# callmeray/PointMVSNet

Hardware: AMD Instinct MI355X
Metric: depth-maps/sec (DTU 640x512, 3 src views, 2 flow iters) (higher is better)
Workload: dtype f32

## Files before the change

pointmvsnet_amd/csrc/conv3d.hip:

```cpp
#include <stdlib.h>

#include "pf_common.h"
#include "pf_bn_resolve.h"

namespace {

typedef float f32x4 __attribute__((ext_vector_type(4)));

struct ConvGeom {
  int Cin, Cout, Di, Hi, Wi, Do, Ho, Wo;
  int ID, IH, IW, IWP, plane;
  int tiles_d, tiles_h, tiles_w;
  int aff_mode, sps, aff_off;
  const float* in_scale;
  const float* in_shift;
  pf_bn_job in_bn;
};

template <int STRIDE, int TD>
struct Stage {
  static constexpr int ID = (TD - 1) * STRIDE + 3;
  static constexpr int IH = 3 * STRIDE + 3;
  static constexpr int IW = 15 * STRIDE + 3;
  static constexpr int IWP = IW + 1;
  static constexpr int RAW = ID * IH * IWP;
  static constexpr int WANT = STRIDE == 1 ? 16 : 17;
  static constexpr int PLANE = RAW + ((WANT - RAW % 32) + 32) % 32;
  static constexpr int ELEMS = ID * IH * IW;
  static constexpr int NXR = (ELEMS + 63) / 64;
};

template <int NT, int STRIDE, int TD, int MINW>
__global__ __launch_bounds__(256, MINW) void conv3d_k3_kernel(const float* __restrict__ x, const float* __restrict__ wp,
                                                        float* __restrict__ y, ConvGeom g,
                                                        double* __restrict__ partials) {
  using St = Stage<STRIDE, TD>;
  constexpr int ID = St::ID, IH = St::IH, IW = St::IW, IWP = St::IWP, PLANE = St::PLANE;
  constexpr int ELEMS = St::ELEMS, NXR = St::NXR;
  constexpr int NCP = NT * 16;
  constexpr int WSZ = 27 * 4 * NCP;
  constexpr int NWR = (WSZ + 255) / 256;
  constexpr int XS = 4 * PLANE;
  extern __shared__ __attribute__((aligned(16))) float lds[];
  float* xs0 = lds;
  float* ws0 = lds + 2 * XS;
  float* tile = lds;
  double* red = reinterpret_cast<double*>(tile + 4 * NCP * 17 + ((4 * NCP * 17) & 1));

  const int tid = threadIdx.x;
  const int wave = __builtin_amdgcn_readfirstlane(tid >> 6), lane = tid & 63;
  const int li = lane & 15, lk = lane >> 4;
  unsigned xb_, xn_;
  pf_xcd_xy<PF_XCD_CONV3D>(xb_, xn_);
  const int n = (int)xn_, bx = (int)xb_;
  const int plane_i = g.Hi * g.Wi, vol_i = plane_i * g.Di;
  const int64_t plane_o = (int64_t)g.Ho * g.Wo, vol_o = plane_o * g.Do;
  const float* xb = x + (int64_t)n * g.Cin * vol_i;
  float* yb = y + (int64_t)n * g.Cout * vol_o;
  const int cgroups = g.Cin >> 2;

  double ssum[NT], ssq[NT];
#pragma unroll
  for (int t = 0; t < NT; ++t) ssum[t] = ssq[t] = 0.0;

  float* aff = lds + g.aff_off;
  if (g.aff_mode == 1) {
    const int stat = n / g.sps;
    for (int e = tid; e < 2 * g.Cin; e += 256)
      aff[e] = e < g.Cin ? g.in_scale[(int64_t)stat * g.Cin + e] : g.in_shift[(int64_t)stat * g.Cin + e - g.Cin];
  } else if (g.aff_mode == 2) {
    pf_bn_resolve<256>(g.in_bn, n / g.sps, aff, aff + g.Cin, reinterpret_cast<double*>(lds));
  }

  const int total = g.tiles_d * g.tiles_h * g.tiles_w;
  for (int item = bx; item < total; item += gridDim.x) {
    const int tw = item % g.tiles_w;
    const int rest = item / g.tiles_w;
    const int th = rest % g.tiles_h;
    const int td = rest / g.tiles_h;
    const int od0 = td * TD, oh0 = th * 4, ow0 = tw * 16;
    const int id0 = od0 * STRIDE - 1, ih0 = oh0 * STRIDE - 1, iw0 = ow0 * STRIDE - 1;

    unsigned gofs[NXR];
    unsigned okmask = 0;
#pragma unroll
    for (int r = 0; r < NXR; ++r) {
      const int e = lane + 64 * r;
      const int row = e / IW, col = e - row * IW;
      const int dz = row / IH, hy = row - dz * IH;
      const int id = id0 + dz, ih = ih0 + hy, iw = iw0 + col;
      const bool ok = e < ELEMS && id >= 0 && id < g.Di && ih >= 0 && ih < g.Hi && iw >= 0 && iw < g.Wi;
      gofs[r] = ok ? (unsigned)(id * plane_i + ih * g.Wi + iw) : 0u;
      okmask |= (ok ? 1u : 0u) << r;
    }

    float rx[NXR], rw[NWR];
    auto load_group = [&](int cg) {
      const float* src = xb + (int64_t)(cg * 4 + wave) * vol_i;
#pragma unroll
      for (int r = 0; r < NXR; ++r) rx[r] = src[gofs[r]];
      const float* wsrc = wp + (int64_t)cg * WSZ;
#pragma unroll
      for (int r = 0; r < NWR; ++r) {
        const int e = tid + 256 * r;
        rw[r] = (256 * (r + 1) <= WSZ || e < WSZ) ? wsrc[e] : 0.0f;
      }
    };
    auto store_group = [&](int buf, int cg) {
      float* xs = xs0 + buf * XS + wave * PLANE;
      float* ws = ws0 + buf * WSZ;
      float sa = 1.0f, sb = 0.0f;
      if (g.aff_mode) {
        sa = aff[cg * 4 + wave];
        sb = aff[g.Cin + cg * 4 + wave];
      }
#pragma unroll
      for (int r = 0; r < NXR; ++r) {
        const int e = lane + 64 * r;
        float v = rx[r];
        if (g.aff_mode) v = fmaxf(fmaf(v, sa, sb), 0.0f);
        if (64 * (r + 1) <= ELEMS || e < ELEMS) xs[e + e / IW] = ((okmask >> r) & 1u) ? v : 0.0f;
      }
#pragma unroll
      for (int r = 0; r < NWR; ++r) {
        const int e = tid + 256 * r;
        if (256 * (r + 1) <= WSZ || e < WSZ) ws[e] = rw[r];
      }
    };

    f32x4 acc[TD][NT];
#pragma unroll
    for (int d = 0; d < TD; ++d)
#pragma unroll
      for (int t = 0; t < NT; ++t) acc[d][t] = (f32x4){0.0f, 0.0f, 0.0f, 0.0f};

    __syncthreads();
    load_group(0);
    store_group(0, 0);
    __syncthreads();
    for (int cg = 0; cg < cgroups; ++cg) {
      const int buf = cg & 1;
      if (cg + 1 < cgroups) load_group(cg + 1);
      const float* xs = xs0 + buf * XS + lk * PLANE + (wave * STRIDE) * IWP + li * STRIDE;
      const float* ws = ws0 + buf * WSZ + lk * NCP + li;
#pragma unroll
      for (int kd = 0; kd < 3; ++kd) {
#pragma unroll
        for (int kh = 0; kh < 3; ++kh) {
#pragma unroll
          for (int kw = 0; kw < 3; ++kw) {
            const int tap = (kd * 3 + kh) * 3 + kw;
            float b[NT];
#pragma unroll
            for (int t = 0; t < NT; ++t) b[t] = ws[tap * 4 * NCP + 16 * t];
#pragma unroll
            for (int d = 0; d < TD; ++d) {
              const float a = xs[((d * STRIDE + kd) * IH + kh) * IWP + kw];
#pragma unroll
              for (int t = 0; t < NT; ++t) acc[d][t] = __builtin_amdgcn_mfma_f32_16x16x4f32(a, b[t], acc[d][t], 0, 0, 0);
            }
          }
        }
      }
      if (cg + 1 < cgroups) store_group(buf ^ 1, cg + 1);
      __syncthreads();
    }

    const int oh = oh0 + wave;
    float* tl = tile + wave * NCP * 17;
#pragma unroll
    for (int d = 0; d < TD; ++d) {
      const int od = od0 + d;
      const bool row_ok = oh < g.Ho && od < g.Do;
#pragma unroll
      for (int t = 0; t < NT; ++t) {
        float s = 0.0f, q = 0.0f;
#pragma unroll
        for (int r = 0; r < 4; ++r) {
          const int pos = lk * 4 + r;
          const float v = acc[d][t][r];
          tl[(16 * t + li) * 17 + pos] = v;
          if (row_ok && ow0 + pos < g.Wo) {
            s += v;
            q += v * v;
          }
        }
        s += __shfl_xor(s, 16);
        q += __shfl_xor(q, 16);
        s += __shfl_xor(s, 32);
        q += __shfl_xor(q, 32);
        ssum[t] += (double)s;
        ssq[t] += (double)q;
      }
      __builtin_amdgcn_wave_barrier();
      if (row_ok) {
        for (int e = lane; e < NCP * 16; e += 64) {
          const int co = e >> 4, pos = e & 15;
          if (co < g.Cout && ow0 + pos < g.Wo)
            yb[(int64_t)co * vol_o + (int64_t)od * plane_o + (int64_t)oh * g.Wo + ow0 + pos] = tl[co * 17 + pos];
        }
      }
      __builtin_amdgcn_wave_barrier();
    }
  }

  if (partials != nullptr) {
#pragma unroll
    for (int t = 0; t < NT; ++t) {
      if (lane < 16) {
        red[((wave * NCP) + 16 * t + lane) * 2 + 0] = ssum[t];
        red[((wave * NCP) + 16 * t + lane) * 2 + 1] = ssq[t];
      }
    }
    __syncthreads();
    if (tid < g.Cout) {
      double s = 0.0, q = 0.0;
#pragma unroll
      for (int w = 0; w < 4; ++w) {
        s += red[((w * NCP) + tid) * 2 + 0];
        q += red[((w * NCP) + tid) * 2 + 1];
      }
      double* o = partials + (((int64_t)n * gridDim.x + bx) * g.Cout + tid) * 2;
      o[0] = s;
      o[1] = q;
    }
  }
}

template <int COUT>
__global__ __launch_bounds__(256) void conv3d_k3_few_kernel(const float* __restrict__ x, const float* __restrict__ w,
                                                            float* __restrict__ y, int Cin, int D, int H, int W) {
  extern __shared__ __attribute__((aligned(16))) float wl[];
  for (int e = threadIdx.x; e < COUT * Cin * 27; e += 256) wl[e] = w[e];
  __syncthreads();
  const int64_t plane = (int64_t)H * W, vol = plane * D;
  const int64_t i = (int64_t)blockIdx.x * 256 + threadIdx.x;
  const int n = blockIdx.y;
  if (i >= vol) return;
  const int od = (int)(i / plane);
  const int rem = (int)(i - (int64_t)od * plane);
  const int oh = rem / W, ow = rem - oh * W;
  float acc[COUT];
#pragma unroll
  for (int c = 0; c < COUT; ++c) acc[c] = 0.0f;
  const float* xb = x + (int64_t)n * Cin * vol;
  for (int ci = 0; ci < Cin; ++ci) {
    const float* xc = xb + (int64_t)ci * vol;
#pragma unroll
    for (int kd = 0; kd < 3; ++kd) {
      const int id = od + kd - 1;
      const bool dok = id >= 0 && id < D;
#pragma unroll
      for (int kh = 0; kh < 3; ++kh) {
        const int ih = oh + kh - 1;
        const bool hok = dok && ih >= 0 && ih < H;
        const float* row = xc + (int64_t)id * plane + (int64_t)ih * W;
#pragma unroll
        for (int kw = 0; kw < 3; ++kw) {
          const int iw = ow + kw - 1;
          const float v = (hok && iw >= 0 && iw < W) ? row[iw] : 0.0f;
#pragma unroll
          for (int c = 0; c < COUT; ++c) acc[c] = fmaf(v, wl[(c * Cin + ci) * 27 + (kd * 3 + kh) * 3 + kw], acc[c]);
        }
      }
    }
  }
#pragma unroll
  for (int c = 0; c < COUT; ++c) y[((int64_t)n * COUT + c) * vol + i] = acc[c];
}

ConvGeom make_geom(int64_t Cin, int64_t Cout, int64_t Di, int64_t Hi, int64_t Wi, int stride, int td) {
  ConvGeom g;
  g.Cin = (int)Cin;
  g.Cout = (int)Cout;
  g.Di = (int)Di;
  g.Hi = (int)Hi;
  g.Wi = (int)Wi;
  g.Do = (int)((Di - 1) / stride + 1);
  g.Ho = (int)((Hi - 1) / stride + 1);
  g.Wo = (int)((Wi - 1) / stride + 1);
  g.ID = (td - 1) * stride + 3;
  g.IH = 3 * stride + 3;
  g.IW = 15 * stride + 3;
  g.IWP = g.IW + 1;
  const int raw = g.ID * g.IH * g.IWP;
  const int want = stride == 1 ? 16 : 17;
  g.plane = raw + ((want - raw % 32) + 32) % 32;
  g.tiles_d = (g.Do + td - 1) / td;
  g.tiles_h = (g.Ho + 3) / 4;
  g.tiles_w = (g.Wo + 15) / 16;
  g.aff_mode = 0;
  g.sps = 1;
  g.aff_off = 0;
  g.in_scale = g.in_shift = nullptr;
  g.in_bn = pf_bn_job{};
  return g;
}

constexpr size_t kMaxLds = 80 * 1024;

size_t lds_work_bytes(const ConvGeom& g, int NT) {
  const int NCP = NT * 16;
  const size_t staging = sizeof(float) * (size_t)(2 * 4 * g.plane + 2 * 27 * 4 * NCP);
  const size_t epilogue = sizeof(float) * (size_t)(4 * NCP * 17 + 1) + sizeof(double) * (size_t)(4 * NCP * 2);
  const size_t m = staging > epilogue ? staging : epilogue;
  return (m + 15) / 16 * 16;
}
size_t lds_bytes_for(const ConvGeom& g, int NT) {
  return lds_work_bytes(g, NT) + sizeof(float) * 2 * (size_t)g.Cin;
}

int pick_td(int64_t Cin, int64_t Cout, int64_t Di, int64_t Hi, int64_t Wi, int stride) {
  const int NT = (int)((Cout + 15) / 16);
  int best = 0;
  for (int td = (stride == 1 && NT > 1) ? 4 : 2; td >= 1; td >>= 1) {
    const ConvGeom g = make_geom(Cin, Cout, Di, Hi, Wi, stride, td);
    if (lds_bytes_for(g, NT) > kMaxLds) continue;
    best = td;
    if ((int64_t)g.tiles_d * g.tiles_h * g.tiles_w >= 512) return td;
  }
  return best;
}

int blocks_for(const ConvGeom& g) {
  const int64_t total = (int64_t)g.tiles_d * g.tiles_h * g.tiles_w;
#ifndef PF_CONV3D_CAP
#define PF_CONV3D_CAP 2048
#endif
  if (total <= PF_CONV3D_CAP) return (int)total;
  const int64_t per = (total + PF_CONV3D_CAP - 1) / PF_CONV3D_CAP;
  return (int)((total + per - 1) / per);
}

template <int NT, int STRIDE, int TD, int MINW>
int launch(const float* x, const float* wp, float* y, const ConvGeom& g, int64_t N, double* partials,
           hipStream_t s) {
  const size_t lds_bytes = lds_bytes_for(g, NT);
  if (lds_bytes > kMaxLds) return PF_ERR_UNSUPPORTED;
  ConvGeom gk = g;
  gk.aff_off = (int)(lds_work_bytes(g, NT) / sizeof(float));
  if (lds_bytes > 64 * 1024) {
    static std::atomic<unsigned long long> done{0};
    const int rc = pf_allow_big_lds(reinterpret_cast<const void*>(&conv3d_k3_kernel<NT, STRIDE, TD, MINW>),
                                    (int)kMaxLds, done);
    if (rc != PF_OK) return rc;
  }
  dim3 grid((unsigned)blocks_for(g), (unsigned)N);
  hipLaunchKernelGGL((conv3d_k3_kernel<NT, STRIDE, TD, MINW>), grid, dim3(256), lds_bytes, s, x, wp, y, gk, partials);
  return pf_launch_status();
}

template <int NT, int STRIDE, int TD>
int launch_w(const float* x, const float* wp, float* y, const ConvGeom& g, int64_t N, double* partials,
             hipStream_t s) {
  constexpr int kDefault = (NT == 1 && STRIDE == 1 && TD == 2) ? 4 : 2;
  return launch<NT, STRIDE, TD, kDefault>(x, wp, y, g, N, partials, s);
}

template <int NT, int STRIDE>
int launch_td(int td, const float* x, const float* wp, float* y, const ConvGeom& g, int64_t N, double* partials,
              hipStream_t s) {
  if constexpr (STRIDE == 1) {
    if (td == 4) return launch_w<NT, STRIDE, 4>(x, wp, y, g, N, partials, s);
  }
  if (td == 2) return launch_w<NT, STRIDE, 2>(x, wp, y, g, N, partials, s);
  return launch_w<NT, STRIDE, 1>(x, wp, y, g, N, partials, s);
}

}

extern "C" {

int pf_conv3d_blocks(int64_t Cin, int64_t Cout, int64_t Di, int64_t Hi, int64_t Wi, int stride) {
  if (Cin <= 0 || Cout <= 0 || Di <= 0 || Hi <= 0 || Wi <= 0 || (stride != 1 && stride != 2)) return 0;
  const int td = pick_td(Cin, Cout, Di, Hi, Wi, stride);
  if (td == 0) return 0;
  return blocks_for(make_geom(Cin, Cout, Di, Hi, Wi, stride, td));
}

int pf_conv3d_k3_f32(const float* x, const float* wp, float* y, int64_t N, int64_t Cin, int64_t Cout, int64_t Di,
                     int64_t Hi, int64_t Wi, int stride, const float* in_scale, const float* in_shift,
                     const pf_bn_job* in_bn, int samples_per_stat, double* partials, void* stream) {
  PF_REQUIRE(N >= 0 && Cin >= 4 && Cout >= 1 && Di >= 1 && Hi >= 1 && Wi >= 1 && N <= 65535);
  PF_REQUIRE(stride == 1 || stride == 2);
  PF_REQUIRE(samples_per_stat >= 1 && (in_scale == nullptr) == (in_shift == nullptr));
  PF_REQUIRE(in_bn == nullptr || in_scale == nullptr);
  if (in_bn != nullptr && N > 0) {
    PF_REQUIRE(N % samples_per_stat == 0);
    const int rc = pf_bn_in_check(in_bn, (int)Cin, (int)(N / samples_per_stat));
    if (rc != PF_OK) return rc;
  }
  if ((Cin % 4) != 0 || Cout > 32) return PF_ERR_UNSUPPORTED;
  PF_REQUIRE(Cin * Di * Hi * Wi <= INT32_MAX);
  if (N == 0) return PF_OK;
  PF_REQUIRE(x && wp && y);
  const int td = pick_td(Cin, Cout, Di, Hi, Wi, stride);
  if (td == 0) return PF_ERR_UNSUPPORTED;
  ConvGeom g = make_geom(Cin, Cout, Di, Hi, Wi, stride, td);
  g.aff_mode = in_bn ? 2 : (in_scale ? 1 : 0);
  g.sps = samples_per_stat;
  g.in_scale = in_scale;
  g.in_shift = in_shift;
  if (in_bn) g.in_bn = *in_bn;
  hipStream_t s = (hipStream_t)stream;
  const int NT = (int)((Cout + 15) / 16);
  if (stride == 1)
    return NT == 1 ? launch_td<1, 1>(td, x, wp, y, g, N, partials, s) : launch_td<2, 1>(td, x, wp, y, g, N, partials, s);
  return NT == 1 ? launch_td<1, 2>(td, x, wp, y, g, N, partials, s) : launch_td<2, 2>(td, x, wp, y, g, N, partials, s);
}

int pf_conv3d_k3_few_f32(const float* x, const float* w, float* y, int64_t N, int64_t Cin, int64_t Cout, int64_t D,
                         int64_t H, int64_t W, void* stream) {
  PF_REQUIRE(N >= 0 && Cin >= 1 && Cout >= 1 && D >= 1 && H >= 1 && W >= 1 && N <= 65535);
  if (Cout > 4 || Cout * Cin * 27 * sizeof(float) > 48 * 1024) return PF_ERR_UNSUPPORTED;
  PF_REQUIRE(H * W <= INT32_MAX);
  if (N == 0) return PF_OK;
  PF_REQUIRE(x && w && y);
  const size_t lds = sizeof(float) * (size_t)(Cout * Cin * 27);
  dim3 grid((unsigned)pf_cdiv(D * H * W, 256), (unsigned)N);
  hipStream_t s = (hipStream_t)stream;
  switch ((int)Cout) {
    case 1: hipLaunchKernelGGL(conv3d_k3_few_kernel<1>, grid, dim3(256), lds, s, x, w, y, (int)Cin, (int)D, (int)H, (int)W); break;
    case 2: hipLaunchKernelGGL(conv3d_k3_few_kernel<2>, grid, dim3(256), lds, s, x, w, y, (int)Cin, (int)D, (int)H, (int)W); break;
    case 3: hipLaunchKernelGGL(conv3d_k3_few_kernel<3>, grid, dim3(256), lds, s, x, w, y, (int)Cin, (int)D, (int)H, (int)W); break;
    default: hipLaunchKernelGGL(conv3d_k3_few_kernel<4>, grid, dim3(256), lds, s, x, w, y, (int)Cin, (int)D, (int)H, (int)W); break;
  }
  return pf_launch_status();
}

}
```

pointmvsnet_amd/csrc/conv3d_bottom.hip:

```cpp
#include <stdlib.h>

#include "pf_common.h"
#include "pf_bn_resolve.h"

namespace {

typedef float f32x4 __attribute__((ext_vector_type(4)));

struct BottomGeom {
  int Di, Hi, Wi, Do, Ho, Wo, tiles_w, sps;
};

template <int CIN, int PD, int PH, int PW, int RS, int AFFINE>
__device__ __forceinline__ void stage_patch3d(const float* __restrict__ xb, int64_t plane_c, int plane_d, int id0,
                                              int ih0, int iw0, int dstep, int Di, int Hi, int Wi, float* patch,
                                              float* aff, const float* __restrict__ in_scale,
                                              const float* __restrict__ in_shift, int stat, const pf_bn_job& in_bn,
                                              double* scratch) {
  constexpr int NPIX = PD * PH * PW;
  constexpr int ITEMS = NPIX * (CIN / 4);
  constexpr int NIT = (ITEMS + 255) / 256;
  const int tid = threadIdx.x;
  float rx[NIT][4];
  bool rok[NIT];
#pragma unroll
  for (int r = 0; r < NIT; ++r) {
    const int it = tid + 256 * r;
    const int itc = it < ITEMS ? it : ITEMS - 1;
    const int q = itc / NPIX, p = itc - q * NPIX;
    const int pd = p / (PH * PW), pp = p - pd * (PH * PW);
    const int pr = pp / PW, pc = pp - pr * PW;
    const int id = id0 + pd * dstep, ih = ih0 + pr, iw = iw0 + pc;
    rok[r] = id >= 0 && id < Di && ih >= 0 && ih < Hi && iw >= 0 && iw < Wi;
    const float* src = xb + (int64_t)(4 * q) * plane_c + (rok[r] ? id * plane_d + ih * Wi + iw : 0);
#pragma unroll
    for (int j = 0; j < 4; ++j) rx[r][j] = src[j * plane_c];
  }
  if (AFFINE == 1) {
    const float* sc = in_scale + (int64_t)stat * CIN;
    const float* sh = in_shift + (int64_t)stat * CIN;
    if (tid < CIN) aff[tid] = sc[tid];
    else if (tid < 2 * CIN) aff[tid] = sh[tid - CIN];
    __syncthreads();
  }
  if (AFFINE == 2) pf_bn_resolve<256>(in_bn, stat, aff, aff + CIN, scratch);
#pragma unroll
  for (int r = 0; r < NIT; ++r) {
    const int it = tid + 256 * r;
    const int itc = it < ITEMS ? it : ITEMS - 1;
    const int q = itc / NPIX, p = itc - q * NPIX;
    f32x4 v = {rx[r][0], rx[r][1], rx[r][2], rx[r][3]};
    if (AFFINE) {
      const f32x4 a = *reinterpret_cast<const f32x4*>(aff + 4 * q);
      const f32x4 b = *reinterpret_cast<const f32x4*>(aff + CIN + 4 * q);
#pragma unroll
      for (int j = 0; j < 4; ++j) v[j] = fmaxf(fmaf(v[j], a[j], b[j]), 0.0f);
    }
    if (!rok[r]) v = (f32x4){0.0f, 0.0f, 0.0f, 0.0f};
    if (256 * (r + 1) <= ITEMS || it < ITEMS) *reinterpret_cast<f32x4*>(patch + p * RS + 4 * q) = v;
  }
}

template <int STRIDE, int CIN>
struct BottomCfg {
  static constexpr int COUT = 64;
  static constexpr int PH = 3 * STRIDE + 3, PW = PH;
  static constexpr int RS = CIN + 4;
  static constexpr int PATCH = 3 * PH * PW * RS;
  static constexpr int KC = CIN / 16;
  static constexpr int STEPS = 27 * KC;
  static constexpr int PF = 32;
  static constexpr size_t LDS = sizeof(float) * (size_t)(PATCH + 1024 + 2 * CIN);
  static_assert(CIN % 16 == 0 && LDS <= 64 * 1024 && STEPS > PF, "shape");
};

template <int STRIDE, int CIN, int AFFINE>
__global__ __launch_bounds__(256) void conv3d_bottom_kernel(const float* __restrict__ x, const float* __restrict__ wp,
                                                            float* __restrict__ y, BottomGeom g,
                                                            const float* __restrict__ in_scale,
                                                            const float* __restrict__ in_shift,
                                                            double* __restrict__ partials, pf_bn_job in_bn) {
  using C = BottomCfg<STRIDE, CIN>;
  constexpr int PH = C::PH, PW = C::PW, RS = C::RS, COUT = 64, KC = C::KC, STEPS = C::STEPS, PF = C::PF;
  extern __shared__ __attribute__((aligned(16))) float lds[];
  float* patch = lds;
  double* scratch = reinterpret_cast<double*>(lds + C::PATCH);
  float* aff = lds + C::PATCH + 1024;

  const int tid = threadIdx.x;
  const int wave = __builtin_amdgcn_readfirstlane(tid >> 6), lane = tid & 63;
  const int li = lane & 15, kq = lane >> 4;
  const int n = blockIdx.z, od = blockIdx.y;
  const int tw = blockIdx.x % g.tiles_w, th = blockIdx.x / g.tiles_w;
  const int oh0 = 4 * th, ow0 = 4 * tw;
  const int plane_d = g.Hi * g.Wi;
  const int64_t plane_c = (int64_t)g.Di * plane_d;
  const float* xb = x + (int64_t)n * CIN * plane_c;

  const f32x4* wg = reinterpret_cast<const f32x4*>(wp) + kq * COUT + 16 * wave + li;
  f32x4 ring[PF];
#pragma unroll
  for (int s = 0; s < PF; ++s) ring[s] = wg[s * 4 * COUT];

  stage_patch3d<CIN, 3, PH, PW, RS, AFFINE>(xb, plane_c, plane_d, od * STRIDE - 1, oh0 * STRIDE - 1, ow0 * STRIDE - 1, 1,
                                            g.Di, g.Hi, g.Wi, patch, aff, in_scale, in_shift, n / g.sps, in_bn, scratch);
  __syncthreads();

  f32x4 acc = {0.0f, 0.0f, 0.0f, 0.0f};
  const float* abase = patch + (((li >> 2) * STRIDE) * PW + (li & 3) * STRIDE) * RS + 4 * kq;
  auto a_ptr = [&](int s) {
    const int tap = s / KC, kc = s - tap * KC;
    const int kd = tap / 9, kh = (tap / 3) % 3, kw = tap % 3;
    return abase + ((kd * PH + kh) * PW + kw) * RS + 16 * kc;
  };
  f32x4 a = *reinterpret_cast<const f32x4*>(a_ptr(0));
#pragma unroll
  for (int s = 0; s < STEPS; ++s) {
    const f32x4 b = ring[s % PF];
    if (s + PF < STEPS) ring[s % PF] = wg[(s + PF) * 4 * COUT];
    f32x4 an = a;
    if (s + 1 < STEPS) an = *reinterpret_cast<const f32x4*>(a_ptr(s + 1));
    __builtin_amdgcn_sched_barrier(0);
#pragma unroll
    for (int j = 0; j < 4; ++j) acc = __builtin_amdgcn_mfma_f32_16x16x4f32(a[j], b[j], acc, 0, 0, 0);
    __builtin_amdgcn_sched_barrier(0);
    a = an;
  }

  const int co = 16 * wave + li;
  const int oh = oh0 + kq;
  float s = 0.0f, q = 0.0f;
  if (oh < g.Ho) {
    float* dst = y + (((int64_t)n * COUT + co) * g.Do + od) * ((int64_t)g.Ho * g.Wo) + (int64_t)oh * g.Wo + ow0;
    if ((g.Wo & 3) == 0) {
      *reinterpret_cast<f32x4*>(dst) = acc;
#pragma unroll
      for (int e = 0; e < 4; ++e) {
        s += acc[e];
        q += acc[e] * acc[e];
      }
    } else {
#pragma unroll
      for (int e = 0; e < 4; ++e)
        if (ow0 + e < g.Wo) {
          dst[e] = acc[e];
          s += acc[e];
          q += acc[e] * acc[e];
        }
    }
  }
  if (partials != nullptr) {
    s += __shfl_xor(s, 16);
    q += __shfl_xor(q, 16);
    s += __shfl_xor(s, 32);
    q += __shfl_xor(q, 32);
    if (lane < 16) {
      double* o = partials + ((((int64_t)n * gridDim.y + od) * gridDim.x + blockIdx.x) * COUT + co) * 2;
      o[0] = (double)s;
      o[1] = (double)q;
    }
  }
}

struct DeconvCfg {
  static constexpr int CIN = 64, COUT = 32, RS = CIN + 4, KC = CIN / 16;
  static constexpr int PATCH = 2 * 5 * 5 * RS;
  static constexpr size_t LDS = sizeof(float) * (size_t)(PATCH + 1024 + 2 * CIN);
};

struct DcItem {
  unsigned char cls, nb, end;
};
__constant__ DcItem kDcItems[4][8] = {
    {{7, 0, 0}, {7, 1, 0}, {7, 2, 0}, {7, 3, 0}, {7, 4, 0}, {7, 5, 0}, {7, 6, 0}, {7, 7, 1}},
    {{3, 0, 0}, {3, 1, 0}, {3, 2, 0}, {3, 3, 1}, {1, 0, 0}, {1, 1, 1}, {0, 0, 0}, {0, 0, 0}},
    {{5, 0, 0}, {5, 1, 0}, {5, 4, 0}, {5, 5, 1}, {2, 0, 0}, {2, 2, 1}, {0, 0, 0}, {0, 0, 0}},
    {{6, 0, 0}, {6, 2, 0}, {6, 4, 0}, {6, 6, 1}, {4, 0, 0}, {4, 4, 1}, {0, 0, 1}, {0, 0, 0}}};
__constant__ int kDcCount[4] = {8, 6, 6, 7};

__device__ __forceinline__ int deconv_tap(int parity, int offset) { return parity == 0 ? 1 : (offset == 1 ? 0 : 2); }

template <int AFFINE>
__global__ __launch_bounds__(256) void deconv3d_bottom_kernel(const float* __restrict__ x, const float* __restrict__ wp,
                                                              float* __restrict__ y, BottomGeom g,
                                                              const float* __restrict__ in_scale,
                                                              const float* __restrict__ in_shift,
                                                              double* __restrict__ partials, pf_bn_job in_bn) {
  using C = DeconvCfg;
  constexpr int RS = C::RS, CIN = C::CIN, COUT = C::COUT, KC = C::KC;
  extern __shared__ __attribute__((aligned(16))) float lds[];
  float* patch = lds;
  double* scratch = reinterpret_cast<double*>(lds + C::PATCH);
  float* aff = lds + C::PATCH + 1024;

  const int tid = threadIdx.x;
  const int wave = __builtin_amdgcn_readfirstlane(tid >> 6), lane = tid & 63;
  const int li = lane & 15, kq = lane >> 4;
  const int n = blockIdx.z, id = blockIdx.y;
  const int tw = blockIdx.x % g.tiles_w, th = blockIdx.x / g.tiles_w;
  const int ih0 = 4 * th, iw0 = 4 * tw;
  const int plane_d = g.Hi * g.Wi;
  const int64_t plane_c = (int64_t)g.Di * plane_d;
  const float* xb = x + (int64_t)n * CIN * plane_c;

  const f32x4* w4 = reinterpret_cast<const f32x4*>(wp) + kq * COUT + li;
  const int nitems = kDcCount[wave];
  auto item_tap = [&](int it) {
    const DcItem d = kDcItems[wave][it];
    const int pd = d.cls >> 2, ph = (d.cls >> 1) & 1, pw = d.cls & 1;
    const int sd = d.nb >> 2, sh = (d.nb >> 1) & 1, sw = d.nb & 1;
    return (deconv_tap(pd, sd) * 3 + deconv_tap(ph, sh)) * 3 + deconv_tap(pw, sw);
  };
  f32x4 bring[3][KC][2];
  auto load_b = [&](int it, f32x4 (*b)[2]) {
    const f32x4* wt = w4 + (int64_t)item_tap(it) * KC * 4 * COUT;
#pragma unroll
    for (int kc = 0; kc < KC; ++kc) {
      b[kc][0] = wt[kc * 4 * COUT];
      b[kc][1] = wt[kc * 4 * COUT + 16];
    }
  };
  load_b(0, bring[0]);
  load_b(1, bring[1]);

  stage_patch3d<CIN, 2, 5, 5, RS, AFFINE>(xb, plane_c, plane_d, id, ih0, iw0, 1, g.Di, g.Hi, g.Wi, patch, aff, in_scale,
                                          in_shift, n / g.sps, in_bn, scratch);
  __syncthreads();

  const float* abase = patch + ((li >> 2) * 5 + (li & 3)) * RS + 4 * kq;
  const int64_t Vo = (int64_t)g.Do * g.Ho * g.Wo;
  const int ih = ih0 + kq;
  double ssum[2] = {0.0, 0.0}, ssq[2] = {0.0, 0.0};
  f32x4 acc[2];
  acc[0] = acc[1] = (f32x4){0.0f, 0.0f, 0.0f, 0.0f};
#pragma unroll
  for (int it = 0; it < 8; ++it) {
    if (it < nitems) {
      if (it + 2 < nitems) load_b(it + 2, bring[(it + 2) % 3]);
      const DcItem d = kDcItems[wave][it];
      const int sd = d.nb >> 2, sh = (d.nb >> 1) & 1, sw = d.nb & 1;
      const float* ap = abase + ((sd * 5 + sh) * 5 + sw) * RS;
      f32x4 a[KC];
#pragma unroll
      for (int kc = 0; kc < KC; ++kc) a[kc] = *reinterpret_cast<const f32x4*>(ap + 16 * kc);
      __builtin_amdgcn_sched_barrier(0);
#pragma unroll
      for (int kc = 0; kc < KC; ++kc)
#pragma unroll
        for (int j = 0; j < 4; ++j) {
          acc[0] = __builtin_amdgcn_mfma_f32_16x16x4f32(a[kc][j], bring[it % 3][kc][0][j], acc[0], 0, 0, 0);
          acc[1] = __builtin_amdgcn_mfma_f32_16x16x4f32(a[kc][j], bring[it % 3][kc][1][j], acc[1], 0, 0, 0);
        }
      __builtin_amdgcn_sched_barrier(0);
      if (d.end) {
        const int pd = d.cls >> 2, ph = (d.cls >> 1) & 1, pw = d.cls & 1;
        if (ih < g.Hi) {
#pragma unroll
          for (int t = 0; t < 2; ++t) {
            float* dst =
                y + ((int64_t)n * COUT + 16 * t + li) * Vo + ((int64_t)(2 * id + pd) * g.Ho + 2 * ih + ph) * g.Wo + pw;
            float s = 0.0f, q = 0.0f;
#pragma unroll
            for (int e = 0; e < 4; ++e)
              if (iw0 + e < g.Wi) {
                dst[2 * (iw0 + e)] = acc[t][e];
                s += acc[t][e];
                q += acc[t][e] * acc[t][e];
              }
            ssum[t] += (double)s;
            ssq[t] += (double)q;
          }
        }
        acc[0] = acc[1] = (f32x4){0.0f, 0.0f, 0.0f, 0.0f};
      }
    }
  }
  if (partials != nullptr) {
    __syncthreads();
    double* red = reinterpret_cast<double*>(patch);
#pragma unroll
    for (int t = 0; t < 2; ++t) {
      double s = ssum[t], q = ssq[t];
      s += __shfl_xor(s, 16);
      q += __shfl_xor(q, 16);
      s += __shfl_xor(s, 32);
      q += __shfl_xor(q, 32);
      if (lane < 16) {
        red[((wave * 32) + 16 * t + lane) * 2 + 0] = s;
        red[((wave * 32) + 16 * t + lane) * 2 + 1] = q;
      }
    }
    __syncthreads();
    if (tid < COUT) {
      double s = 0.0, q = 0.0;
#pragma unroll
      for (int w = 0; w < 4; ++w) {
        s += red[(w * 32 + tid) * 2 + 0];
        q += red[(w * 32 + tid) * 2 + 1];
      }
      double* o = partials + ((((int64_t)n * gridDim.y + id) * gridDim.x + blockIdx.x) * COUT + tid) * 2;
      o[0] = s;
      o[1] = q;
    }
  }
}

template <int STRIDE, int CIN, int AFFINE>
int launch_bottom_mode(const float* x, const float* wp, float* y, BottomGeom g, int64_t N, const float* in_scale,
                       const float* in_shift, double* partials, const pf_bn_job& in_bn, hipStream_t s) {
  using C = BottomCfg<STRIDE, CIN>;
  g.tiles_w = (g.Wo + 3) / 4;
  dim3 grid((unsigned)(((g.Ho + 3) / 4) * g.tiles_w), (unsigned)g.Do, (unsigned)N);
  hipLaunchKernelGGL((conv3d_bottom_kernel<STRIDE, CIN, AFFINE>), grid, dim3(256), C::LDS, s, x, wp, y, g, in_scale,
                     in_shift, partials, in_bn);
  return pf_launch_status();
}

template <int STRIDE, int CIN>
int launch_bottom(const float* x, const float* wp, float* y, BottomGeom g, int64_t N, const float* in_scale,
                  const float* in_shift, double* partials, const pf_bn_job* in_bn, hipStream_t s) {
  pf_bn_job none = {};
  if (in_bn != nullptr) {
    const int rc = pf_bn_in_check(in_bn, CIN, (int)(N / g.sps));
    if (rc != PF_OK) return rc;
    return launch_bottom_mode<STRIDE, CIN, 2>(x, wp, y, g, N, nullptr, nullptr, partials, *in_bn, s);
  }
  if (in_scale != nullptr) return launch_bottom_mode<STRIDE, CIN, 1>(x, wp, y, g, N, in_scale, in_shift, partials, none, s);
  return launch_bottom_mode<STRIDE, CIN, 0>(x, wp, y, g, N, nullptr, nullptr, partials, none, s);
}

template <int AFFINE>
int launch_deconv_mode(const float* x, const float* wp, float* y, BottomGeom g, int64_t N, const float* in_scale,
                       const float* in_shift, double* partials, const pf_bn_job& in_bn, hipStream_t s) {
  g.tiles_w = (g.Wi + 3) / 4;
  dim3 grid((unsigned)(((g.Hi + 3) / 4) * g.tiles_w), (unsigned)g.Di, (unsigned)N);
  hipLaunchKernelGGL((deconv3d_bottom_kernel<AFFINE>), grid, dim3(256), DeconvCfg::LDS, s, x, wp, y, g, in_scale,
                     in_shift, partials, in_bn);
  return pf_launch_status();
}

}

extern "C" {

int pf_conv3d_bottom_supported(int64_t Cin, int64_t Cout, int stride) {
  return Cout == 64 && ((stride == 1 && Cin == 64) || (stride == 2 && Cin == 32));
}

int pf_conv3d_bottom_blocks(int64_t Di, int64_t Hi, int64_t Wi, int stride) {
  if (Di <= 0 || Hi <= 0 || Wi <= 0 || (stride != 1 && stride != 2)) return 0;
  const int64_t Do = (Di - 1) / stride + 1, Ho = (Hi - 1) / stride + 1, Wo = (Wi - 1) / stride + 1;
  return (int)(Do * ((Ho + 3) / 4) * ((Wo + 3) / 4));
}

int pf_conv3d_bottom_f32(const float* x, const float* wp, float* y, int64_t N, int64_t Cin, int64_t Cout, int64_t Di,
                         int64_t Hi, int64_t Wi, int stride, const float* in_scale, const float* in_shift,
                         const pf_bn_job* in_bn, int samples_per_stat, double* partials, void* stream) {
  PF_REQUIRE(N >= 0 && Cin >= 1 && Cout >= 1 && Di >= 1 && Hi >= 1 && Wi >= 1 && N <= 65535 && samples_per_stat >= 1);
  PF_REQUIRE((in_scale == nullptr) == (in_shift == nullptr) && (in_bn == nullptr || in_scale == nullptr));
  PF_REQUIRE(N % samples_per_stat == 0 || in_bn == nullptr);
  if (!pf_conv3d_bottom_supported(Cin, Cout, stride)) return PF_ERR_UNSUPPORTED;
  PF_REQUIRE(Di * Hi * Wi <= INT32_MAX / 4 && Di <= 65535);
  if (N == 0) return PF_OK;
  PF_REQUIRE(x && wp && y);
  BottomGeom g;
  g.Di = (int)Di;
  g.Hi = (int)Hi;
  g.Wi = (int)Wi;
  g.Do = (int)((Di - 1) / stride + 1);
  g.Ho = (int)((Hi - 1) / stride + 1);
  g.Wo = (int)((Wi - 1) / stride + 1);
  g.tiles_w = 0;
  g.sps = samples_per_stat;
  hipStream_t s = (hipStream_t)stream;
  if (stride == 1) return launch_bottom<1, 64>(x, wp, y, g, N, in_scale, in_shift, partials, in_bn, s);
  return launch_bottom<2, 32>(x, wp, y, g, N, in_scale, in_shift, partials, in_bn, s);
}

int pf_deconv3d_bottom_supported(int64_t Cin, int64_t Cout) { return Cin == 64 && Cout == 32; }

int pf_deconv3d_bottom_blocks(int64_t Di, int64_t Hi, int64_t Wi) {
  if (Di <= 0 || Hi <= 0 || Wi <= 0) return 0;
  return (int)(Di * ((Hi + 3) / 4) * ((Wi + 3) / 4));
}

int pf_deconv3d_bottom_f32(const float* x, const float* wp, float* y, int64_t N, int64_t Cin, int64_t Cout, int64_t Di,
                           int64_t Hi, int64_t Wi, const float* in_scale, const float* in_shift, const pf_bn_job* in_bn,
                           int samples_per_stat, double* partials, void* stream) {
  PF_REQUIRE(N >= 0 && Cin >= 1 && Cout >= 1 && Di >= 1 && Hi >= 1 && Wi >= 1 && N <= 65535 && samples_per_stat >= 1);
  PF_REQUIRE((in_scale == nullptr) == (in_shift == nullptr) && (in_bn == nullptr || in_scale == nullptr));
  PF_REQUIRE(N % samples_per_stat == 0 || in_bn == nullptr);
  if (!pf_deconv3d_bottom_supported(Cin, Cout)) return PF_ERR_UNSUPPORTED;
  PF_REQUIRE(Di * Hi * Wi <= INT32_MAX / 32 && Di <= 65535);
  if (N == 0) return PF_OK;
  PF_REQUIRE(x && wp && y);
  BottomGeom g;
  g.Di = (int)Di;
  g.Hi = (int)Hi;
  g.Wi = (int)Wi;
  g.Do = (int)(2 * Di);
  g.Ho = (int)(2 * Hi);
  g.Wo = (int)(2 * Wi);
  g.tiles_w = 0;
  g.sps = samples_per_stat;
  hipStream_t s = (hipStream_t)stream;
  pf_bn_job none = {};
  if (in_bn != nullptr) {
    const int rc = pf_bn_in_check(in_bn, 64, (int)(N / samples_per_stat));
    if (rc != PF_OK) return rc;
    return launch_deconv_mode<2>(x, wp, y, g, N, nullptr, nullptr, partials, *in_bn, s);
  }
  if (in_scale != nullptr) return launch_deconv_mode<1>(x, wp, y, g, N, in_scale, in_shift, partials, none, s);
  return launch_deconv_mode<0>(x, wp, y, g, N, nullptr, nullptr, partials, none, s);
}

}
```

Baseline: 1105.

## Add small-volume MFMA conv3d kernel for Cout=32 layers with few tiles

Measured after the change: 1112 (median of 6 runs). Within noise of the previous version (+0.7%).

```diff
diff --git a/pointmvsnet_amd/csrc/conv3d.hip b/pointmvsnet_amd/csrc/conv3d.hip
--- a/pointmvsnet_amd/csrc/conv3d.hip
+++ b/pointmvsnet_amd/csrc/conv3d.hip
@@ -2,6 +2,7 @@
 
 #include "pf_common.h"
 #include "pf_bn_resolve.h"
+#include "pf_patch3d.h"
 
 namespace {
 
@@ -267,6 +268,111 @@
   }
 #pragma unroll
   for (int c = 0; c < COUT; ++c) y[((int64_t)n * COUT + c) * vol + i] = acc[c];
+}
+
+template <int STRIDE, int CIN>
+struct SmallCfg {
+  static constexpr int COUT = 32, TDZ = 2;
+  static constexpr int PD = (TDZ - 1) * STRIDE + 3, PH = 3 * STRIDE + 3, PW = PH;
+  static constexpr int RS = CIN + 4;
+  static constexpr int PATCH = PD * PH * PW * RS;
+  static constexpr int KC = CIN / 16;
+  static constexpr int STEPS = 27 * KC;
+  static constexpr int PF = STEPS < 32 ? STEPS : 32;
+  static constexpr size_t LDS = sizeof(float) * (size_t)(PATCH + 1024 + 2 * CIN);
+  static_assert(CIN % 16 == 0 && LDS <= 64 * 1024, "shape");
+};
+
+template <int STRIDE, int CIN, int AFFINE>
+__global__ __launch_bounds__(256) void conv3d_k3_small_kernel(const float* __restrict__ x, const float* __restrict__ wp,
+                                                              float* __restrict__ y, ConvGeom g,
+                                                              double* __restrict__ partials) {
+  using C = SmallCfg<STRIDE, CIN>;
+  constexpr int PH = C::PH, PW = C::PW, RS = C::RS, COUT = C::COUT, KC = C::KC, STEPS = C::STEPS, PF = C::PF;
+  extern __shared__ __attribute__((aligned(16))) float lds[];
+  float* patch = lds;
+  double* scratch = reinterpret_cast<double*>(lds + C::PATCH);
+  float* aff = lds + C::PATCH + 1024;
+
+  const int tid = threadIdx.x;
+  const int wave = __builtin_amdgcn_readfirstlane(tid >> 6), lane = tid & 63;
+  const int li = lane & 15, kq = lane >> 4;
+  const int cgw = wave & 1, dz = wave >> 1;
+  const int n = blockIdx.z, od0 = blockIdx.y * C::TDZ;
+  const int tw = blockIdx.x % g.tiles_w, th = blockIdx.x / g.tiles_w;
+  const int oh0 = 4 * th, ow0 = 4 * tw;
+  const int plane_d = g.Hi * g.Wi;
+  const int64_t plane_c = (int64_t)g.Di * plane_d;
+  const float* xb = x + (int64_t)n * CIN * plane_c;
+
+  const float* wg = wp + (int64_t)kq * (27 * 4 * COUT) + 16 * cgw + li;
+  auto load_b = [&](int s) {
+    const int tap = s / KC, kc = s - tap * KC;
+    const float* src = wg + (kc * 4 * 27 + tap) * (4 * COUT);
+    return (f32x4){src[0], src[COUT], src[2 * COUT], src[3 * COUT]};
+  };
+  f32x4 ring[PF];
+#pragma unroll
+  for (int s = 0; s < PF; ++s) ring[s] = load_b(s);
+
+  pf_stage_patch3d<CIN, C::PD, PH, PW, RS, AFFINE>(xb, plane_c, plane_d, od0 * STRIDE - 1, oh0 * STRIDE - 1,
+                                                   ow0 * STRIDE - 1, 1, g.Di, g.Hi, g.Wi, patch, aff, g.in_scale,
+                                                   g.in_shift, n / g.sps, g.in_bn, scratch);
+  __syncthreads();
+
+  f32x4 acc = {0.0f, 0.0f, 0.0f, 0.0f};
+  const float* abase = patch + (((dz * STRIDE) * PH + (li >> 2) * STRIDE) * PW + (li & 3) * STRIDE) * RS + 4 * kq;
+  auto a_ptr = [&](int s) {
+    const int tap = s / KC, kc = s - tap * KC;
+    const int kd = tap / 9, kh = (tap / 3) % 3, kw = tap % 3;
+    return abase + ((kd * PH + kh) * PW + kw) * RS + 16 * kc;
+  };
+  f32x4 a = *reinterpret_cast<const f32x4*>(a_ptr(0));
+#pragma unroll
+  for (int s = 0; s < STEPS; ++s) {
+    const f32x4 b = ring[s % PF];
+    if (s + PF < STEPS) ring[s % PF] = load_b(s + PF);
+    f32x4 an = a;
+    if (s + 1 < STEPS) an = *reinterpret_cast<const f32x4*>(a_ptr(s + 1));
+    __builtin_amdgcn_sched_barrier(0);
+#pragma unroll
+    for (int j = 0; j < 4; ++j) acc = __builtin_amdgcn_mfma_f32_16x16x4f32(a[j], b[j], acc, 0, 0, 0);
+    __builtin_amdgcn_sched_barrier(0);
+    a = an;
+  }
+
+  const int co = 16 * cgw + li;
+  const int od = od0 + dz, oh = oh0 + kq;
+  double s = 0.0, q = 0.0;
+  if (od < g.Do && oh < g.Ho) {
+    float* dst = y + (((int64_t)n * COUT + co) * g.Do + od) * ((int64_t)g.Ho * g.Wo) + (int64_t)oh * g.Wo + ow0;
+    if ((g.Wo & 3) == 0) *reinterpret_cast<f32x4*>(dst) = acc;
+#pragma unroll
+    for (int e = 0; e < 4; ++e)
+      if (ow0 + e < g.Wo) {
+        if ((g.Wo & 3) != 0) dst[e] = acc[e];
+        s += (double)acc[e];
+        q += (double)acc[e] * (double)acc[e];
+      }
+  }
+  if (partials != nullptr) {
+    s += __shfl_xor(s, 16);
+    q += __shfl_xor(q, 16);
+    s += __shfl_xor(s, 32);
+    q += __shfl_xor(q, 32);
+    double* red = scratch;
+    if (lane < 16) {
+      red[(dz * COUT + co) * 2 + 0] = s;
+      red[(dz * COUT + co) * 2 + 1] = q;
+    }
+    __syncthreads();
+    if (tid < 2 * COUT) {
+      double v = 0.0;
+#pragma unroll
+      for (int d = 0; d < C::TDZ; ++d) v += red[d * COUT * 2 + tid];
+      partials[(((int64_t)n * gridDim.y + blockIdx.y) * gridDim.x + blockIdx.x) * COUT * 2 + tid] = v;
+    }
+  }
 }
 
 ConvGeom make_geom(int64_t Cin, int64_t Cout, int64_t Di, int64_t Hi, int64_t Wi, int stride, int td) {
@@ -367,6 +473,29 @@
   return launch_w<NT, STRIDE, 1>(x, wp, y, g, N, partials, s);
 }
 
+bool small_form(int64_t Cin, int64_t Cout, int64_t Di, int64_t Hi, int64_t Wi, int stride, int td) {
+  if (Cout != 32 || (Cin != 16 && Cin != 32) || td == 0) return false;
+  const ConvGeom g = make_geom(Cin, Cout, Di, Hi, Wi, stride, td);
+  return (int64_t)g.tiles_d * g.tiles_h * g.tiles_w < 256;
+}
+
+template <int STRIDE, int CIN, int AFFINE>
+int launch_small_mode(const float* x, const float* wp, float* y, const ConvGeom& g, int64_t N, double* partials,
+                      hipStream_t s) {
+  using C = SmallCfg<STRIDE, CIN>;
+  dim3 grid((unsigned)(((g.Ho + 3) / 4) * g.tiles_w), (unsigned)((g.Do + C::TDZ - 1) / C::TDZ), (unsigned)N);
+  hipLaunchKernelGGL((conv3d_k3_small_kernel<STRIDE, CIN, AFFINE>), grid, dim3(256), C::LDS, s, x, wp, y, g, partials);
+  return pf_launch_status();
+}
+
+template <int STRIDE, int CIN>
+int launch_small(const float* x, const float* wp, float* y, ConvGeom g, int64_t N, double* partials, hipStream_t s) {
+  g.tiles_w = (g.Wo + 3) / 4;
+  if (g.aff_mode == 2) return launch_small_mode<STRIDE, CIN, 2>(x, wp, y, g, N, partials, s);
+  if (g.aff_mode == 1) return launch_small_mode<STRIDE, CIN, 1>(x, wp, y, g, N, partials, s);
+  return launch_small_mode<STRIDE, CIN, 0>(x, wp, y, g, N, partials, s);
+}
+
 }
 
 extern "C" {
@@ -375,7 +504,9 @@
   if (Cin <= 0 || Cout <= 0 || Di <= 0 || Hi <= 0 || Wi <= 0 || (stride != 1 && stride != 2)) return 0;
   const int td = pick_td(Cin, Cout, Di, Hi, Wi, stride);
   if (td == 0) return 0;
-  return blocks_for(make_geom(Cin, Cout, Di, Hi, Wi, stride, td));
+  const ConvGeom g = make_geom(Cin, Cout, Di, Hi, Wi, stride, td);
+  if (small_form(Cin, Cout, Di, Hi, Wi, stride, td)) return ((g.Do + 1) / 2) * ((g.Ho + 3) / 4) * ((g.Wo + 3) / 4);
+  return blocks_for(g);
 }
 
 int pf_conv3d_k3_f32(const float* x, const float* wp, float* y, int64_t N, int64_t Cin, int64_t Cout, int64_t Di,
@@ -403,6 +534,12 @@
   g.in_shift = in_shift;
   if (in_bn) g.in_bn = *in_bn;
   hipStream_t s = (hipStream_t)stream;
+  if (small_form(Cin, Cout, Di, Hi, Wi, stride, td)) {
+    PF_REQUIRE(g.Do <= 2 * 65535);
+    if (stride == 1)
+      return Cin == 16 ? launch_small<1, 16>(x, wp, y, g, N, partials, s) : launch_small<1, 32>(x, wp, y, g, N, partials, s);
+    return Cin == 16 ? launch_small<2, 16>(x, wp, y, g, N, partials, s) : launch_small<2, 32>(x, wp, y, g, N, partials, s);
+  }
   const int NT = (int)((Cout + 15) / 16);
   if (stride == 1)
     return NT == 1 ? launch_td<1, 1>(td, x, wp, y, g, N, partials, s) : launch_td<2, 1>(td, x, wp, y, g, N, partials, s);
diff --git a/pointmvsnet_amd/csrc/conv3d_bottom.hip b/pointmvsnet_amd/csrc/conv3d_bottom.hip
--- a/pointmvsnet_amd/csrc/conv3d_bottom.hip
+++ b/pointmvsnet_amd/csrc/conv3d_bottom.hip
@@ -2,6 +2,7 @@
 
 #include "pf_common.h"
 #include "pf_bn_resolve.h"
+#include "pf_patch3d.h"
 
 namespace {
 
@@ -10,56 +11,6 @@
 struct BottomGeom {
   int Di, Hi, Wi, Do, Ho, Wo, tiles_w, sps;
 };
-
-template <int CIN, int PD, int PH, int PW, int RS, int AFFINE>
-__device__ __forceinline__ void stage_patch3d(const float* __restrict__ xb, int64_t plane_c, int plane_d, int id0,
-                                              int ih0, int iw0, int dstep, int Di, int Hi, int Wi, float* patch,
-                                              float* aff, const float* __restrict__ in_scale,
-                                              const float* __restrict__ in_shift, int stat, const pf_bn_job& in_bn,
-                                              double* scratch) {
-  constexpr int NPIX = PD * PH * PW;
-  constexpr int ITEMS = NPIX * (CIN / 4);
-  constexpr int NIT = (ITEMS + 255) / 256;
-  const int tid = threadIdx.x;
-  float rx[NIT][4];
-  bool rok[NIT];
-#pragma unroll
-  for (int r = 0; r < NIT; ++r) {
-    const int it = tid + 256 * r;
-    const int itc = it < ITEMS ? it : ITEMS - 1;
-    const int q = itc / NPIX, p = itc - q * NPIX;
-    const int pd = p / (PH * PW), pp = p - pd * (PH * PW);
-    const int pr = pp / PW, pc = pp - pr * PW;
-    const int id = id0 + pd * dstep, ih = ih0 + pr, iw = iw0 + pc;
-    rok[r] = id >= 0 && id < Di && ih >= 0 && ih < Hi && iw >= 0 && iw < Wi;
-    const float* src = xb + (int64_t)(4 * q) * plane_c + (rok[r] ? id * plane_d + ih * Wi + iw : 0);
-#pragma unroll
-    for (int j = 0; j < 4; ++j) rx[r][j] = src[j * plane_c];
-  }
-  if (AFFINE == 1) {
-    const float* sc = in_scale + (int64_t)stat * CIN;
-    const float* sh = in_shift + (int64_t)stat * CIN;
-    if (tid < CIN) aff[tid] = sc[tid];
-    else if (tid < 2 * CIN) aff[tid] = sh[tid - CIN];
-    __syncthreads();
-  }
-  if (AFFINE == 2) pf_bn_resolve<256>(in_bn, stat, aff, aff + CIN, scratch);
-#pragma unroll
-  for (int r = 0; r < NIT; ++r) {
-    const int it = tid + 256 * r;
-    const int itc = it < ITEMS ? it : ITEMS - 1;
-    const int q = itc / NPIX, p = itc - q * NPIX;
-    f32x4 v = {rx[r][0], rx[r][1], rx[r][2], rx[r][3]};
-    if (AFFINE) {
-      const f32x4 a = *reinterpret_cast<const f32x4*>(aff + 4 * q);
-      const f32x4 b = *reinterpret_cast<const f32x4*>(aff + CIN + 4 * q);
-#pragma unroll
-      for (int j = 0; j < 4; ++j) v[j] = fmaxf(fmaf(v[j], a[j], b[j]), 0.0f);
-    }
-    if (!rok[r]) v = (f32x4){0.0f, 0.0f, 0.0f, 0.0f};
-    if (256 * (r + 1) <= ITEMS || it < ITEMS) *reinterpret_cast<f32x4*>(patch + p * RS + 4 * q) = v;
-  }
-}
 
 template <int STRIDE, int CIN>
 struct BottomCfg {
@@ -102,7 +53,7 @@
 #pragma unroll
   for (int s = 0; s < PF; ++s) ring[s] = wg[s * 4 * COUT];
 
-  stage_patch3d<CIN, 3, PH, PW, RS, AFFINE>(xb, plane_c, plane_d, od * STRIDE - 1, oh0 * STRIDE - 1, ow0 * STRIDE - 1, 1,
+  pf_stage_patch3d<CIN, 3, PH, PW, RS, AFFINE>(xb, plane_c, plane_d, od * STRIDE - 1, oh0 * STRIDE - 1, ow0 * STRIDE - 1, 1,
                                             g.Di, g.Hi, g.Wi, patch, aff, in_scale, in_shift, n / g.sps, in_bn, scratch);
   __syncthreads();
 
@@ -223,7 +174,7 @@
   load_b(0, bring[0]);
   load_b(1, bring[1]);
 
-  stage_patch3d<CIN, 2, 5, 5, RS, AFFINE>(xb, plane_c, plane_d, id, ih0, iw0, 1, g.Di, g.Hi, g.Wi, patch, aff, in_scale,
+  pf_stage_patch3d<CIN, 2, 5, 5, RS, AFFINE>(xb, plane_c, plane_d, id, ih0, iw0, 1, g.Di, g.Hi, g.Wi, patch, aff, in_scale,
                                           in_shift, n / g.sps, in_bn, scratch);
   __syncthreads();
 
diff --git a/pointmvsnet_amd/csrc/pf_patch3d.h b/pointmvsnet_amd/csrc/pf_patch3d.h
--- /dev/null
+++ b/pointmvsnet_amd/csrc/pf_patch3d.h
@@ -0,0 +1,58 @@
+#pragma once
+
+#include "pf_common.h"
+#include "pf_bn_resolve.h"
+
+#if defined(__HIPCC__)
+typedef float pf_f32x4 __attribute__((ext_vector_type(4)));
+
+template <int CIN, int PD, int PH, int PW, int RS, int AFFINE>
+__device__ __forceinline__ void pf_stage_patch3d(const float* __restrict__ xb, int64_t plane_c, int plane_d, int id0,
+                                              int ih0, int iw0, int dstep, int Di, int Hi, int Wi, float* patch,
+                                              float* aff, const float* __restrict__ in_scale,
+                                              const float* __restrict__ in_shift, int stat, const pf_bn_job& in_bn,
+                                              double* scratch) {
+  constexpr int NPIX = PD * PH * PW;
+  constexpr int ITEMS = NPIX * (CIN / 4);
+  constexpr int NIT = (ITEMS + 255) / 256;
+  const int tid = threadIdx.x;
+  float rx[NIT][4];
+  bool rok[NIT];
+#pragma unroll
+  for (int r = 0; r < NIT; ++r) {
+    const int it = tid + 256 * r;
+    const int itc = it < ITEMS ? it : ITEMS - 1;
+    const int q = itc / NPIX, p = itc - q * NPIX;
+    const int pd = p / (PH * PW), pp = p - pd * (PH * PW);
+    const int pr = pp / PW, pc = pp - pr * PW;
+    const int id = id0 + pd * dstep, ih = ih0 + pr, iw = iw0 + pc;
+    rok[r] = id >= 0 && id < Di && ih >= 0 && ih < Hi && iw >= 0 && iw < Wi;
+    const float* src = xb + (int64_t)(4 * q) * plane_c + (rok[r] ? id * plane_d + ih * Wi + iw : 0);
+#pragma unroll
+    for (int j = 0; j < 4; ++j) rx[r][j] = src[j * plane_c];
+  }
+  if (AFFINE == 1) {
+    const float* sc = in_scale + (int64_t)stat * CIN;
+    const float* sh = in_shift + (int64_t)stat * CIN;
+    if (tid < CIN) aff[tid] = sc[tid];
+    else if (tid < 2 * CIN) aff[tid] = sh[tid - CIN];
+    __syncthreads();
+  }
+  if (AFFINE == 2) pf_bn_resolve<256>(in_bn, stat, aff, aff + CIN, scratch);
+#pragma unroll
+  for (int r = 0; r < NIT; ++r) {
+    const int it = tid + 256 * r;
+    const int itc = it < ITEMS ? it : ITEMS - 1;
+    const int q = itc / NPIX, p = itc - q * NPIX;
+    pf_f32x4 v = {rx[r][0], rx[r][1], rx[r][2], rx[r][3]};
+    if (AFFINE) {
+      const pf_f32x4 a = *reinterpret_cast<const pf_f32x4*>(aff + 4 * q);
+      const pf_f32x4 b = *reinterpret_cast<const pf_f32x4*>(aff + CIN + 4 * q);
+#pragma unroll
+      for (int j = 0; j < 4; ++j) v[j] = fmaxf(fmaf(v[j], a[j], b[j]), 0.0f);
+    }
+    if (!rok[r]) v = (pf_f32x4){0.0f, 0.0f, 0.0f, 0.0f};
+    if (256 * (r + 1) <= ITEMS || it < ITEMS) *reinterpret_cast<pf_f32x4*>(patch + p * RS + 4 * q) = v;
+  }
+}
+#endif
```
